# mhnazeri/PMoE

Hardware: AMD Instinct MI355X
Metric: samples/sec fwd+bwd, 256x256 RGB 4-expert PMoE (higher is better)
Workload: dtype bf16; 1 GPU; 4-expert MoE (PMoE experts), 256x256x3 x4 frames, batch 64/GPU, fwd+moe_loss+bwd, dropout 0.3; global_batch=64, parallelism=dp1

## Files before the change

### include/pmoe_hip.h

```cpp
#ifndef PMOE_HIP_H
#define PMOE_HIP_H
#include <stdint.h>
#ifdef __cplusplus
extern "C" {
#endif

#define PMOE_DT_BF16 0
#define PMOE_DT_F32 1

#define PMOE_ERR_ARG (-1)
#define PMOE_ERR_UNSUPPORTED (-2)

#define PMOE_ACT_NONE 0
#define PMOE_ACT_RELU 1
#define PMOE_ACT_ELU 2
#define PMOE_ACT_TANH 3
#define PMOE_ACT_SIGMOID 4

#define PMOE_RES_NONE 0
#define PMOE_RES_ADD 1
#define PMOE_RES_DRELU 2
#define PMOE_RES_DELU 3
#define PMOE_RES_DTANH 4
#define PMOE_RES_DSIGMOID 5
// ... 98 lines not shown
                  int64_t rows_per_expert, int32_t E, int32_t C, int32_t relu, int32_t y_ld, int32_t y_coff,
                  int32_t dtype, void* y_fp8, float in_scale, void* stream);
int pmoe_bn_apply_gap(const void* x, void* y, const float* scale, const float* shift, const float* mean, float* gap_part,
                      int32_t nparts, int32_t N, int32_t ipe, int64_t HW, int32_t C, int32_t relu, int32_t dtype, void* stream);
int pmoe_bn_bwd_reduce(const void* dy, const void* y, const void* x, const float* mean, const float* invstd,
                       const float* scale, const float* shift, int64_t rows_per_expert, int32_t E, int32_t C, int32_t relu, float* part, int32_t nparts,
                       void* gmask_out, int32_t dtype, void* stream);
int pmoe_bn_bwd_finalize(const float* part, int32_t nparts, int64_t count, float* dgamma, float* dbeta, float* c1,
                         float* c2, int32_t E, int32_t C, void* stream);
int pmoe_bn_apply_pool2(const void* x, void* y, void* pooled, const float* scale, const float* shift, const float* mean,
                        int32_t ipe, int32_t H, int32_t W, int32_t E, int32_t C, int32_t relu, int32_t y_ld, int32_t y_coff,
                        int32_t dtype, void* stream);
int pmoe_bn_bwd_apply(const void* dy, const void* y, const void* x, const float* mean, const float* invstd,
                      const float* scale, const float* shift, const float* c1, const float* c2, void* dx, void* gmask_out,
                      int64_t rows_per_expert, int32_t E, int32_t C, int32_t relu, int32_t dtype, void* stream);

int pmoe_maxpool3s2_fwd(const void* x, void* y, uint8_t* argmax, int32_t N, int32_t H, int32_t W, int32_t C,
                        int32_t dtype, void* stream);
int pmoe_maxpool3s2_bwd(const void* dy, const uint8_t* argmax, void* dx, int32_t N, int32_t H, int32_t W, int32_t C,
                        int32_t dtype, void* stream);
int pmoe_gap_partial(const void* a, const void* b, float* part, int32_t N, int64_t HW, int32_t C, int32_t nparts,
                     int32_t b_shared_ipe, int32_t dtype, void* stream);
int pmoe_gap_finish(const float* part, void* out, int32_t N, int32_t C, int32_t nparts, int64_t HW, int32_t out_ld,
                    int32_t out_coff, int32_t dtype, void* stream);
int pmoe_gap_bwd(const void* g, void* dx, int32_t N, int64_t HW, int32_t C, int32_t g_ld, int32_t g_coff,
                 int32_t dtype, void* stream);

int pmoe_stem_tail_stats(const void* z2, const float* sc2, const float* sh2, const float* mu2, float* part,
                         int32_t nparts, float* shiftc, float* part_x, int32_t E, int32_t ipe, int32_t H, int32_t W,
                         int32_t C, int32_t dtype, void* stream);
// ... 126 lines not shown
```

### pmoe_amd/csrc/elementwise.hip

```cpp
#include "common.h"

#define DISPATCH_DT(dtype, CALL)                      \
    do {                                              \
        if ((dtype) == PMOE_DT_BF16) { using T = bf16; CALL; } \
        else if ((dtype) == PMOE_DT_F32) { using T = float; CALL; } \
        else return PMOE_ERR_ARG;                     \
    } while (0)

static inline bool pow2(int v) { return v > 0 && !(v & (v - 1)); }

template <typename T, int MODE>
__global__ void __launch_bounds__(256) colstats_kernel(const T* __restrict__ x, const T* __restrict__ dy,
                                                      const T* __restrict__ y, const float* __restrict__ mean,
                                                      const float* __restrict__ invstd, const float* __restrict__ scale,
                                                      const float* __restrict__ shift, long long rpe, int C, int ld,
                                                      int coff, int relu, float* __restrict__ part, int nparts,
                                                      float* __restrict__ shiftc, T* __restrict__ gmask) {
    constexpr int VE = 16 / (int)sizeof(T);
    const int CV = C / VE, RL = 256 / CV;
    const int tid = threadIdx.x, cv = tid % CV, rl = tid / CV;
    const int e = blockIdx.y, pi = blockIdx.x;
    const long long rpp = (rpe + nparts - 1) / nparts;
    long long r0 = (long long)pi * rpp, r1 = r0 + rpp;
    if (r1 > rpe) r1 = rpe;
// ... 258 lines not shown
            for (int k = 0; k < VE; ++k) gv[k] = ((xv[k] - mu[k]) * sc[k] + sh[k]) > 0.f ? gv[k] : 0.f;
        } else if (relu) {
            float yv[VE];
            unpack16<T>(ldg16(y + off), yv);
#pragma unroll
            for (int k = 0; k < VE; ++k) gv[k] = yv[k] > 0.f ? gv[k] : 0.f;
        }
#pragma unroll
        for (int k = 0; k < VE; ++k) o[k] = gv[k] * A[k] + ((xv[k] - mu[k]) * Bx[k] + K[k]);
        stg16(dx + off, pack16<T>(o));
        if (gm) stg16(gm + off, pack16<T>(gv));
    }
}

template <typename T>
__global__ void __launch_bounds__(256) bn_apply_pool2_kernel(const T* __restrict__ x, T* __restrict__ y, T* __restrict__ pooled,
                                                            const float* __restrict__ scale, const float* __restrict__ shift,
                                                            const float* __restrict__ mean, int ipe, int H, int W, int C, int relu,
                                                            int y_ld, int y_coff) {
    constexpr int VE = 16 / (int)sizeof(T);
    const int CV = C / VE;
    const int e = blockIdx.y, Ho = H / 2, Wo = W / 2;
    const long long nq = (long long)ipe * Ho * Wo * CV;
    const long long i0 = (long long)blockIdx.x * 256 + threadIdx.x;
    const int cv = (int)(i0 % CV);
    float sc[VE], sh[VE], mu[VE];
#pragma unroll
    for (int k = 0; k < VE; ++k) {
        sc[k] = scale[e * C + cv * VE + k]; sh[k] = shift[e * C + cv * VE + k]; mu[k] = mean[e * C + cv * VE + k];
    }
// ... 500 lines not shown
                      const float* scale, const float* shift, const float* c1, const float* c2, void* dx, void* gmask_out,
                      int64_t rows_per_expert, int32_t E, int32_t C, int32_t relu, int32_t dtype, void* stream) {
    DISPATCH_DT(dtype, {
        constexpr int VE = 16 / (int)sizeof(T);
        if (C % VE || !pow2(C / VE) || C / VE > 256) return PMOE_ERR_ARG;
        const long long nvec = rows_per_expert * (C / VE);
        int cap = 1024 / (E > 0 ? E : 1);
        cap = cap < 64 ? 64 : cap;
        hipLaunchKernelGGL((bn_bwd_apply_kernel<T>), dim3(grid_for(nvec, cap), E), dim3(256), 0, (hipStream_t)stream,
                           (const T*)dy, (const T*)y, (const T*)x, mean, invstd, scale, shift, c1, c2, (T*)dx, (T*)gmask_out,
                           (long long)rows_per_expert, C, relu);
        return (int)hipGetLastError();
    });
}

int pmoe_act_fwd(const void* x, void* y, int64_t n, int32_t act, float drop_p, uint64_t seed, int32_t dtype, void* stream) {
    if (!x || !y || n <= 0 || act < PMOE_ACT_NONE || act > PMOE_ACT_SIGMOID || drop_p < 0.f || drop_p >= 1.f) return PMOE_ERR_ARG;
    DISPATCH_DT(dtype, {
        constexpr int VE = 16 / (int)sizeof(T);
        if (n % VE) return PMOE_ERR_ARG;
        hipLaunchKernelGGL((act_fwd_kernel<T>), dim3(grid_for(n / VE)), dim3(256), 0, (hipStream_t)stream, (const T*)x, (T*)y,
                           (long long)(n / VE), act, drop_p, (unsigned long long)seed);
        return (int)hipGetLastError();
    });
}

int pmoe_act_bwd(const void* dy, const void* y, void* dx, int64_t n, int32_t act, float drop_p, int32_t dtype, void* stream) {
    if (!dy || !y || !dx || n <= 0 || act < PMOE_ACT_NONE || act > PMOE_ACT_SIGMOID || drop_p < 0.f || drop_p >= 1.f) return PMOE_ERR_ARG;
    DISPATCH_DT(dtype, {
        constexpr int VE = 16 / (int)sizeof(T);
// ... 144 lines not shown
```

### pmoe_amd/engine.py

```python
import itertools
import os

import torch
import torch.distributed as dist

from . import hip, ops
from .model import blocks as B
from .parallel import BucketedAllReduce

F32 = torch.float32


def r16(c):
    return (c + 15) // 16 * 16


def r64(c):
    return (c + 63) // 64 * 64


class Var:
    __slots__ = ("t", "coff", "c", "g", "needs_grad", "act", "drop_p", "base", "gap_part", "bn_src", "bn_part", "f8", "bn_defer",
                 "bn_fused", "pending_bn")

    def __init__(self, t, c=None, coff=0, needs_grad=False, base=None):
        self.t, self.coff, self.c = t, coff, (c if c is not None else t.shape[-1])
        self.g, self.needs_grad, self.act, self.drop_p, self.base = None, needs_grad, hip.ACT_NONE, 0.0, base
        self.gap_part = None
        self.bn_src = None
        self.bn_part = None
        self.f8 = None
        self.bn_defer = False
        self.bn_fused = None
        self.pending_bn = None

    @property
    def grad(self):
        return self.base.g if self.base is not None else self.g

    def set_grad(self, g):
        if (self.base if self.base is not None else self).bn_part is not None:
            raise RuntimeError("relu(BatchNorm(z)) whose backward reductions came out of its consumer's data gradient "
                               "(PMOE_RES_DBN) must have exactly one consumer; a second gradient contribution arrived "
                               "(set PMOE_BN_REDUCE_IN_DGRAD=0 for graphs that fan this activation out)")
        if self.base is not None:
            self.base.g = g
        else:
            self.g = g

# ... 139 lines not shown
        self._built_for = self._ptr_key = self._packed_version = None
        self._build_gen = 0
        self._seed_counter = itertools.count(1)
        self.fuse_conv_stats = True
        self.fuse_stem_tail = True
        self.fold_stem_input = True
        self.overlap_wgrad = os.environ.get("PMOE_OVERLAP_WGRAD", "0") == "1"
        self.fold_bn_eval = True
        self.pooled_stem_bwd = True
        self.fold_eca_gate = True
        self.bn_mask_in_reduce = os.environ.get("PMOE_BN_MASK_IN_REDUCE", "1") != "0"
        self.bn_reduce_in_dgrad = os.environ.get("PMOE_BN_REDUCE_IN_DGRAD", "1") != "0"
        self.fuse_bn_gap = os.environ.get("PMOE_FUSE_BN_GAP", "1") != "0"
        self.stem_bn_fuse = os.environ.get("PMOE_STEM_BN_FUSE", "1") != "0"
        self.mlp_wgrad_fused = os.environ.get("PMOE_MLP_WGRAD", "1") != "0"
        self.fp8 = False
        self.fp8_in_scale = 16.0
        self.fp8_min_cin = int(os.environ.get("PMOE_FP8_MIN_CIN", "64"))
        self.raw_alpha = False
        self.debug_grads = None
        self.debug_acts = None
        self._collect()

    def _collect(self):
        ex = self.experts
        self.params = []
        self.all_convs = []

        def conv(name, mods, ks=None):
            m0 = mods[0]
# ... 334 lines not shown
            if part is None:
                nparts = self._nparts(rpe)
                part = torch.empty(E, nparts, 2, C_, dtype=F32, device=self.dev)
                shiftc = torch.empty(E, C_, dtype=F32, device=self.dev)
                ops.colstats(rpe, z.t, E, C_, part, nparts, shiftc=shiftc)
            part, nparts = self._fold_parts(part, nparts, 2 * C_, cap=2048)
            ops.bn_finalize(part, nparts, rpe, self._tab("gamma", layer), self._tab("beta", layer),
                            self._tab("rm", layer), self._tab("rv", layer), layer.momentum, layer.eps, True, scale,
                            shift, mean, invstd, E, C_, shiftc)
            self._bn_touched.append(layer)
        else:
            ops.bn_finalize(scale, 0, rpe, self._tab("gamma", layer), self._tab("beta", layer), self._tab("rm", layer),
                            self._tab("rv", layer), layer.momentum, layer.eps, False, scale, shift, mean, invstd, E, C_)
        return scale, shift, mean, invstd

    def _bn(self, z, layer, relu, res=None, stats=None, out=None, out_coff=0, want_gap=False, want_f8=False, pool_to=None):
        E, C_ = self.E, layer.C
        n, h, w, _ = z.t.shape
        rpe = self.B * h * w
        if stats is not None and stats.shape[2] != C_:
            raise RuntimeError("fused stats width mismatch")
        scale, shift, mean, invstd = self._bn_coeffs(layer, rpe, stats, stats.shape[0] // E if stats is not None else 0, z)
        if out is None:
            y = Var(torch.empty_like(z.t))
        elif self.taping:
            y = Var(out.t, C_, out_coff)
        else:
            y = out.window(out_coff, C_)
        ops.set_meta(name=layer.name, bytes=z.t.numel() * z.t.element_size() * (3 if res is not None else 2))
        if want_gap and res is None and out is None and self.fuse_bn_gap:
            nparts = self._gap_parts(h * w)
            part = torch.empty(n, nparts, C_, dtype=F32, device=self.dev)
            ops.bn_apply_gap(z.t, y.t, scale, shift, mean, part, nparts, self.B, relu)
            y.gap_part = (part, nparts)
        elif pool_to is not None and res is None:
            ops.bn_apply_pool2(z.t, y.t, pool_to, scale, shift, mean, self.B, E, C_, relu, y_coff=y.coff)
        else:
            if want_f8 and out is None and self.dtype == torch.bfloat16:
                y.f8 = torch.empty(y.t.shape, dtype=torch.uint8, device=self.dev)
            ops.bn_apply(z.t, res.t if res is not None else None, y.t, scale, shift, mean, rpe, E, C_, relu, y_coff=y.coff,
                         y_fp8=y.f8, in_scale=self.fp8_in_scale)
        if self.debug_acts is not None and relu:
            self.debug_acts[layer.name] = (y.t, y.coff, C_)
        if (relu and res is None and out is None and self.taping and self.training and self.bn_reduce_in_dgrad
                and self.dtype == torch.bfloat16 and z.needs_grad):
            y.bn_src = (z, layer, self._last_coef, rpe)
        y.needs_grad = z.needs_grad or layer.trainable or (res is not None and res.needs_grad)
        if out is not None and y.needs_grad:
            out.needs_grad = True
        if self.taping and y.needs_grad:
            train = self.training
            self.tape.append(lambda: self._bn_bwd(z, layer, y, res, relu, scale, shift, mean, invstd, rpe, train))
        return y

    def _bn_bwd(self, z, layer, y, res, relu, scale, shift, mean, invstd, rpe, train):
        dy = y.grad
# ... 10 lines not shown
                raise RuntimeError("BatchNorm reductions from the data-gradient epilogue: channel count mismatch")
            part, nparts = self._fold_parts(part.view(E, nparts, 2 * C_), nparts, 2 * C_, cap=2048)
            c1, c2 = self._bn_bwd_finalize(layer, part, nparts, rpe, train)
            if z.needs_grad:
                if z.grad is not None:
                    raise RuntimeError("BN input consumed twice")
                if z.bn_defer:
                    z.bn_fused = (dy, y.bn_src[2], c1, c2)
                    z.set_grad(dy)
                    return
                dz = torch.empty_like(z.t)
                ops.set_meta(name=layer.name, bytes=nb * 3)
                ops.bn_bwd_apply(dy, None, z.t, mean, invstd, scale, shift, c1, c2, dz, None, rpe, E, C_, False)
                z.set_grad(dz)
            return
        nparts = self._nparts(rpe)
        part = torch.empty(E, nparts, 2, C_, dtype=F32, device=self.dev)
        want_res = res is not None and res.needs_grad
        gm = torch.empty_like(z.t) if (want_res and relu and ysrc is not None and self.bn_mask_in_reduce) else None
        ops.set_meta(name=layer.name, bytes=nb * ((3 if ysrc is not None else 2) + (gm is not None)))
        ops.bn_bwd_reduce(dy, ysrc, z.t, mean, invstd, scale, shift, rpe, E, C_, relu, part, nparts, gmask=gm)
        part, nparts = self._fold_parts(part, nparts, 2 * C_, cap=2048)
        c1, c2 = self._bn_bwd_finalize(layer, part, nparts, rpe, train)
        dz = torch.empty_like(z.t) if z.needs_grad else None
        if gm is not None:
            if dz is not None:
                ops.set_meta(name=layer.name, bytes=nb * 3)
                ops.bn_bwd_apply(gm, None, z.t, mean, invstd, scale, shift, c1, c2, dz, None, rpe, E, C_, False)
        else:
            gm = torch.empty_like(z.t) if want_res else None
# ... 2 lines not shown
            if dz is None:
                dz = torch.empty_like(z.t)
            ops.set_meta(name=layer.name, bytes=nb * (2 + (ysrc is not None) + 1 + (gm is not None)))
            ops.bn_bwd_apply(dy, ysrc, z.t, mean, invstd, scale, shift, c1, c2, dz, gm, rpe, E, C_, relu)
        if self.debug_grads is not None:
            self.debug_grads[layer.name + ":dz"] = dz.detach().clone()
            self.debug_grads[layer.name + ":stats"] = (mean.clone(), invstd.clone(), c1.clone(), c2.clone())
        if z.needs_grad:
            if z.grad is not None:
                raise RuntimeError("BN input consumed twice")
            z.set_grad(dz)
        if want_res:
            if res.grad is not None:
                raise RuntimeError("residual gradient slot already filled")
            res.set_grad(gm)

    def _bn_bwd_finalize(self, layer, part, nparts, rpe, train, out=None):
        E, C_ = self.E, layer.C
        c1, c2 = out or (torch.empty(E, C_, dtype=F32, device=self.dev) for _ in range(2))
        dgamma, dbeta, store = self._bn_grad_views(layer)
        ops.bn_bwd_finalize(part, nparts, rpe, dgamma, dbeta, c1, c2, E, C_)
        if store is not None:
            store()
        if not train:
            c1.zero_()
            c2.zero_()
        return c1, c2

    def _bn_grad_views(self, layer):
        return (self._grad_slot("gamma", layer).view(self.E, layer.C), self._grad_slot("beta", layer).view(self.E, layer.C),
# ... 327 lines not shown
            a1 = self._conv_bn(x0s, self.conv1, self.bn_c1, relu=True)
        if fold2:
            z2, st = self._eca_conv_folded(a1, self.eca2, self.conv2)
        else:
            a1s = self._eca(a1, self.eca2, shared=False)
            z2, st = self._conv_stats(a1s, self.conv2)
        if self.fuse_stem_tail:
            o = self._stem_tail(z2, st)
        else:
            a2 = self._bn(z2, self.bn_c2, relu=True, stats=st)
            a3 = self._bn(a2, self.bn1, relu=True)
            o = self._maxpool(a3)
        for bi, blk in enumerate(self.blocks):
            idn = o
            if blk["down"] is not None:
                idn = self._conv_bn(o, blk["down"][0], blk["down"][1], relu=False)
            nxt = self.blocks[bi + 1]["conv1"] if bi + 1 < len(self.blocks) else None
            aA = self._conv_bn(o, blk["conv1"], blk["bn1"], relu=True, want_f8=blk["conv2"].fp8)
            o = self._conv_bn(aA, blk["conv2"], blk["bn2"], relu=True, res=idn, want_f8=nxt is not None and nxt.fp8)
        self._gap_to(o, feat, 0)

    def _conv_bn(self, x, conv, bn, relu, res=None, out=None, want_f8=False, pool_to=None):
        if self.training or self.taping or not self.fold_bn_eval or conv.w_f8 is not None:
            z, st = self._conv_stats(x, conv)
            return self._bn(z, bn, relu=relu, res=res, stats=st, out=out, want_f8=want_f8, pool_to=pool_to)
        E = self.E
        key = (self.dtype, str(self.dev)) + tuple(p._version for p in conv.weights) + tuple(
            v for m in bn.mods for v in (m.weight._version, m.bias._version, m.running_mean._version, m.running_var._version))
        cache = conv.__dict__.get("_bn_fold")
        if cache is None or cache[0] != key:
            scale, shift, mean, _ = self._bn_coeffs(bn, 1)
            wf = torch.empty(E, conv.coutp, conv.taps, conv.cinp, dtype=self.dtype, device=self.dev)
            bf = torch.empty(E, conv.coutp, dtype=F32, device=self.dev)
            ops.pack_conv_weights_scaled(self._tab("w", conv), scale, shift, mean, wf, bf, E, conv.cout, conv.cin, conv.ks,
                                         conv.coutp, conv.cinp, self.dtype)
            cache = conv.__dict__["_bn_fold"] = (key, wf, bf)
        _, wf, bf = cache
        Ho, Wo, o = self._conv_out(x, conv, out)
        ops.set_meta(flop=2.0 * self.N * Ho * Wo * conv.cout * conv.cin * conv.taps, name=conv.name + "+bn")
        ops.conv2d(x.t, wf, o.t, cin=conv.cinp, cout=conv.cout_st, coutp=conv.coutp, ipe=self.B, ks=conv.ks,
# ... 173 lines not shown
```

### pmoe_amd/engine_punet.py

```python
import os
import types

import torch

from . import hip, ops
from .engine import ExpertGroupEngine, GroupedBN, GroupedConv, Var, r16, F32


class _UpConv(GroupedConv):
    route_bias = False

    def __init__(self, eng, name, mod):
        super().__init__(eng, name, None, None, mod.in_channels, 4 * mod.out_channels, 1, 1, 0)
        self.mod, self.c_up = mod, mod.out_channels
        self.need_dgrad = False
        self.biases = [mod.bias]
        self._derived_version = None

    @property
    def trainable(self):
        return self.mod.weight.requires_grad or self.mod.bias.requires_grad

    def scatter_grads(self, eng, full_w, full_b):
        eng._grad_slot("wT", self).view(self.cin, self.c_up, 2, 2).copy_(
# ... 10 lines not shown
                              self.cinp, self.dg_rows, self.dg_red, self.w_fwd.dtype)
        ops.pack_bias(hip.ptr_table([b], dev), self.bias_packed, 1, self.cout, self.coutp)
        self._derived_version = ver


class PUNetEngine(ExpertGroupEngine):
    _punet_trains = False

    def __init__(self, expert, return_inter=None):
        self.return_inter = expert.return_inter if return_inter is None else return_inter
        self._punet_built_for, self._punet_build_gen = None, 0
        self.debug_pass_out = self.debug_forced_masks = None
        self.debug_x0 = self.debug_x0_kept = None
        self.debug_keep_x0 = False
        super().__init__([expert], alt=False)

    def _collect_pre_backbone(self, ex):
        pu = ex[0].punet
        self.pu = pu
        self.up_layers = []
        self.shadow_bns = []
        self.unet = self._collect_unet("punet.unet", pu.unet)
        conv, bn, eca = self._mk["conv"], self._mk["bn"], self._mk["eca"]
        eb = pu.entry_block
        self.entry = dict(eca1=eca("punet.entry.eca1", [eb.layer1.eca1]),
                          conv1=conv("punet.entry.conv1", [eb.layer1.conv1[0]]),
                          bn1=bn("punet.entry.bn1", [eb.layer1.conv1[1]]),
                          eca2=eca("punet.entry.eca2", [eb.layer2.eca2]),
                          conv2=conv("punet.entry.conv2", [eb.layer2.conv2[0]]),
                          bn2=self._padded_bn("punet.entry.bn2", eb.layer2.conv2[1]))
# ... 604 lines not shown
```

### pmoe_amd/hip.py

```python
import ctypes as C
import os
from pathlib import Path

import torch

_LIB_PATH = Path(os.environ.get("PMOE_HIP_LIB") or Path(__file__).resolve().parent / "libpmoe_hip.so")
_lib = None

ABI_VERSION = 401
DT_BF16, DT_F32 = 0, 1
ACT_NONE, ACT_RELU, ACT_ELU, ACT_TANH, ACT_SIGMOID = 0, 1, 2, 3, 4
RES_NONE, RES_ADD, RES_DRELU, RES_DELU, RES_DTANH, RES_DSIGMOID, RES_DBN, RES_INBN = 0, 1, 2, 3, 4, 5, 6, 7
ERR_ARG, ERR_UNSUPPORTED = -1, -2
RES_OF_ACT = {ACT_RELU: RES_DRELU, ACT_ELU: RES_DELU, ACT_TANH: RES_DTANH, ACT_SIGMOID: RES_DSIGMOID}
ACT_BY_NAME = {"relu": ACT_RELU, "elu": ACT_ELU, "tanh": ACT_TANH, "sigmoid": ACT_SIGMOID}

_TORCH_DT = {torch.bfloat16: DT_BF16, torch.float32: DT_F32}


class HipUnavailable(RuntimeError):
    pass


class ConvDesc(C.Structure):
# ... 46 lines not shown
    "pmoe_pack_conv_weights": [_P, _P, _P, _I, _I, _I, _I, _I, _I, _I, _I, _I, _P],
    "pmoe_pack_conv_weights_fp8": [_P, _P, _P, _P, _P, _F, _I, _I, _I, _I, _I, _I, _I, _I, _P],
    "pmoe_pack_conv_weights_scaled": [_P, _P, _P, _P, _P, _P, _I, _I, _I, _I, _I, _I, _I, _P],
    "pmoe_pack_conv_weights_gated": [_P, _P, _I, _P, _P, _I, _I, _I, _I, _I, _I, _I, _I, _I, _I, _P],
    "pmoe_unpack_conv_wgrad": [_P, _P, _I, _I, _I, _I, _I, _I, _P],
    "pmoe_pack_bias": [_P, _P, _I, _I, _I, _P],
    "pmoe_act_fwd": [_P, _P, _L, _I, _F, C.c_uint64, _I, _P],
    "pmoe_act_bwd": [_P, _P, _P, _L, _I, _F, _I, _P],
    "pmoe_colstats": [_P, _L, _I, _I, _I, _I, _P, _I, _P, _I, _P],
    "pmoe_reduce_partials": [_P, _P, _I, _I, _I, _I, _P],
    "pmoe_bn_finalize": [_P, _I, _L, _P, _P, _P, _P, _F, _F, _I, _P, _P, _P, _P, _I, _I, _P, _P],
    "pmoe_bn_apply": [_P, _P, _P, _P, _P, _P, _L, _I, _I, _I, _I, _I, _I, _P, _F, _P],
    "pmoe_bn_bwd_reduce": [_P, _P, _P, _P, _P, _P, _P, _L, _I, _I, _I, _P, _I, _P, _I, _P],
    "pmoe_bn_bwd_finalize": [_P, _I, _L, _P, _P, _P, _P, _I, _I, _P],
    "pmoe_bn_bwd_apply": [_P, _P, _P, _P, _P, _P, _P, _P, _P, _P, _P, _L, _I, _I, _I, _I, _P],
    "pmoe_stem_tail_stats": [_P, _P, _P, _P, _P, _I, _P, _P, _I, _I, _I, _I, _I, _I, _P],
    "pmoe_stem_tail_pooled": [_P, _P, _P, C.POINTER(C.c_void_p), _P, _I, _I, _L, _I, _I, _P],
    "pmoe_stem_tail_combine": [_P, _I, _P, _I, C.POINTER(C.c_void_p), _L, _P, _P, _I, _I, _P],
    "pmoe_stem_tail_pool": [_P, _P, _P, _P, _P, _P, _P, _P, _P, _I, _I, _I, _I, _I, _I, _P],
    "pmoe_stem_tail_bwd": [_I, _P, _P, _P, _P, C.POINTER(C.c_void_p), _P, _I, _I, _I, _I, _I, _I, _I, _P],
    "pmoe_maxpool3s2_fwd": [_P, _P, _P, _I, _I, _I, _I, _I, _P],
    "pmoe_maxpool3s2_bwd": [_P, _P, _P, _I, _I, _I, _I, _I, _P],
    "pmoe_gap_partial": [_P, _P, _P, _I, _L, _I, _I, _I, _I, _P],
    "pmoe_bn_apply_gap": [_P, _P, _P, _P, _P, _P, _I, _I, _I, _L, _I, _I, _I, _P],
    "pmoe_gap_finish": [_P, _P, _I, _I, _I, _L, _I, _I, _I, _P],
    "pmoe_gap_bwd": [_P, _P, _I, _L, _I, _I, _I, _I, _P],
    "pmoe_eca_gate": [_P, _I, _L, _P, _I, _P, _P, _I, _I, _I, _I, _I, _P],
    "pmoe_eca_scale": [_P, _P, _P, _I, _L, _I, _I, _I, _P],
    "pmoe_eca_bwd_small": [_P, _I, _P, _P, _P, _I, _P, _P, _P, _I, _I, _I, _I, _F, _P],
    "pmoe_eca_stem_fold": [_P, _P, _P, _P, _P, _I, _I, _I, _I, _I, _I, _I, _I, _P],
# ... 148 lines not shown
```

### pmoe_amd/ops.py

```python
import ctypes as C

import torch

from . import hip
from .hip import ConvDesc, WgradDesc, check, dt, load, ptr, stream_ptr


def _round_up(v, m):
    return (v + m - 1) // m * m


def conv_out_size(h, ks, stride, pad):
    return (h + 2 * pad - ks) // stride + 1


def _nhwc(t, name):
    if t.dim() != 4:
        raise ValueError(f"{name}: expected NHWC [N,H,W,C], got shape {tuple(t.shape)}")
    return t.shape


def _conv_desc(n, h, w_, ho, wo, cin, cout, coutp, ipe, ks, stride, pad, dtype, *, dilate=False, in_shared=False, in_ld=0,
               in_coff=0, out_ld=0, out_coff=0, res_mode=hip.RES_NONE, res_ld=0, res_coff=0, act=hip.ACT_NONE, drop_p=0.0, seed=0,
               w_fp8=False, in_fp8=False, in_scale=1.0, bn_ipe=0, shuffle2_c=0):
# ... 264 lines not shown
                                    ptr(scale), ptr(shift), rpe, E, C_, int(relu), ptr(part, "part", torch.float32), nparts,
                                    ptr(gmask, "gmask", dy.dtype), dt(dy), stream_ptr()), "pmoe_bn_bwd_reduce")


def bn_bwd_finalize(part, nparts, count, dgamma, dbeta, c1, c2, E, C_):
    check(load().pmoe_bn_bwd_finalize(ptr(part), nparts, count, ptr(dgamma), ptr(dbeta), ptr(c1), ptr(c2), E, C_,
                                      stream_ptr()), "pmoe_bn_bwd_finalize")


def bn_bwd_apply(dy, y, x, mean, invstd, scale, shift, c1, c2, dx, gmask, rpe, E, C_, relu):
    check(load().pmoe_bn_bwd_apply(ptr(dy, "dy"), ptr(y, "y", dy.dtype), ptr(x, "x", dy.dtype), ptr(mean), ptr(invstd),
                                   ptr(scale), ptr(shift), ptr(c1), ptr(c2), ptr(dx, "dx", dy.dtype), ptr(gmask, "gmask", dy.dtype),
                                   rpe, E, C_, int(relu), dt(dy), stream_ptr()), "pmoe_bn_bwd_apply")


def stem_tail_stats(z2, sc2, sh2, mu2, part, nparts, E, ipe, shiftc=None, part_x=None):
    n, h, w_, c = _nhwc(z2, "z2")
    check(load().pmoe_stem_tail_stats(ptr(z2, "z2"), ptr(sc2), ptr(sh2), ptr(mu2), ptr(part, "part", torch.float32), nparts,
                                      ptr(shiftc, "shiftc", torch.float32), ptr(part_x, "part_x", torch.float32), E, ipe,
                                      h, w_, c, dt(z2), stream_ptr()), "pmoe_stem_tail_stats")


def _consts12(consts):
    return (C.c_void_p * 12)(*[t.data_ptr() if t is not None else None for t in consts])


def stem_tail_pooled(y, dpool, argmax, consts, part4, nparts, E):
    n, ho, wo, c = _nhwc(y, "y")
    check(load().pmoe_stem_tail_pooled(ptr(y, "y"), ptr(dpool, "dpool", y.dtype), ptr(argmax, "argmax", torch.uint8),
                                       _consts12(consts), ptr(part4, "part4", torch.float32), nparts, E,
# ... 164 lines not shown
        meta, _next_meta = _next_meta, {}
        e0, e1 = torch.cuda.Event(enable_timing=True), torch.cuda.Event(enable_timing=True)
        e0.record()
        r = fn(*a, **k)
        e1.record()
        if _launch_info:
            meta.update(_launch_info)
            _launch_info.clear()
        _prof.append((fn.__name__, meta, e0, e1))
        return r
    return wrapper


for _n in ("stem_tail_stats", "stem_tail_pool", "stem_tail_bwd", "stem_tail_pooled", "stem_tail_combine", "conv2d", "conv2d_wgrad", "conv2d_wgrad_fold", "pack_conv_weights", "pack_conv_weights_scaled", "pack_conv_weights_gated", "unpack_conv_wgrad", "pack_bias", "colstats",
           "reduce_partials", "bn_finalize", "bn_apply", "bn_apply_gap", "bn_bwd_reduce", "bn_bwd_finalize", "bn_bwd_apply",
           "maxpool_fwd", "maxpool_bwd", "gap_partial", "gap_finish", "gap_bwd", "eca_gate", "eca_scale",
           "eca_bwd_small", "eca_bwd_apply", "eca_stem_fold", "nchw_to_nhwc", "pad_rows", "gate_mixture_fwd", "gate_mixture_bwd",
           "moe_loss"):
    globals()[_n] = _timed(globals()[_n])


def maxpool2_fwd(x, y, c=None, x_coff=0):
    n, h, w_, ld = _nhwc(x, "x")
    c = ld if c is None else c
    if tuple(y.shape) != (n, h // 2, w_ // 2, c):
        raise ValueError(f"maxpool2_fwd: y must be {(n, h // 2, w_ // 2, c)}, got {tuple(y.shape)}")
    check(load().pmoe_maxpool2s2_fwd(ptr(x, "x"), ptr(y, "y", x.dtype), n, h, w_, c, ld, x_coff, dt(x), stream_ptr()),
          "pmoe_maxpool2s2_fwd")


# ... 217 lines not shown
```

Baseline: 1953 samples/s.

## Fold shortcut downsample BatchNorm into residual block's BN apply and backward

Defers the downsample-branch BatchNorm during training, so the shortcut's normalized tensor is never materialized. The block's second BN applies both normalizations in one pass (bn_apply_pair). Backward uses paired reduce and apply kernels that compute both BNs' gradient statistics and input gradients from one read of the shared masked gradient. This removes a separate BN apply pass plus one backward pass and several launches per downsample block. The cost is more registers and shared memory per kernel, and tighter shape constraints enforced at runtime.

```diff
diff --git a/include/pmoe_hip.h b/include/pmoe_hip.h
--- a/include/pmoe_hip.h
+++ b/include/pmoe_hip.h
@@ -136,6 +136,16 @@
 int pmoe_bn_bwd_apply(const void* dy, const void* y, const void* x, const float* mean, const float* invstd,
                       const float* scale, const float* shift, const float* c1, const float* c2, void* dx, void* gmask_out,
                       int64_t rows_per_expert, int32_t E, int32_t C, int32_t relu, int32_t dtype, void* stream);
+int pmoe_bn_apply_pair(const void* x, const void* xd, void* y, const float* scale, const float* shift, const float* mean,
+                       const float* scale_d, const float* shift_d, const float* mean_d, int64_t rows_per_expert, int32_t E,
+                       int32_t C, int32_t relu, int32_t dtype, void* y_fp8, float in_scale, void* stream);
+int pmoe_bn_bwd_reduce_pair(const void* dy, const void* y, const void* x, const void* xd, const float* mean,
+                            const float* invstd, const float* mean_d, const float* invstd_d, int64_t rows_per_expert, int32_t E,
+                            int32_t C, float* part, float* part_d, int32_t nparts, void* gmask_out, int32_t dtype, void* stream);
+int pmoe_bn_bwd_apply_pair(const void* g, const void* x, const void* xd, const float* mean, const float* invstd,
+                           const float* scale, const float* c1, const float* c2, const float* mean_d, const float* invstd_d,
+                           const float* scale_d, const float* c1_d, const float* c2_d, void* dx, void* dxd,
+                           int64_t rows_per_expert, int32_t E, int32_t C, int32_t dtype, void* stream);
 
 int pmoe_maxpool3s2_fwd(const void* x, void* y, uint8_t* argmax, int32_t N, int32_t H, int32_t W, int32_t C,
                         int32_t dtype, void* stream);
diff --git a/pmoe_amd/csrc/elementwise.hip b/pmoe_amd/csrc/elementwise.hip
--- a/pmoe_amd/csrc/elementwise.hip
+++ b/pmoe_amd/csrc/elementwise.hip
@@ -296,6 +296,164 @@
 }
 
 template <typename T>
+__global__ void __launch_bounds__(256) bn_apply_pair_kernel(const T* __restrict__ x, const T* __restrict__ xd, T* __restrict__ y,
+                                                           const float* __restrict__ scale, const float* __restrict__ shift,
+                                                           const float* __restrict__ mean, const float* __restrict__ scale_d,
+                                                           const float* __restrict__ shift_d, const float* __restrict__ mean_d,
+                                                           long long rpe, int C, int relu, unsigned char* __restrict__ y8,
+                                                           float in_scale) {
+    constexpr int VE = 16 / (int)sizeof(T);
+    const int CV = C / VE;
+    const int e = blockIdx.y;
+    const long long nvec = rpe * CV;
+    const size_t ebase = (size_t)e * rpe * C;
+    const long long i0 = (long long)blockIdx.x * 256 + threadIdx.x;
+    const int cv = (int)(i0 % CV);
+    float sc[VE], sh[VE], mu[VE], scd[VE], shd[VE], mud[VE];
+#pragma unroll
+    for (int k = 0; k < VE; ++k) {
+        const int c = e * C + cv * VE + k;
+        sc[k] = scale[c]; sh[k] = shift[c]; mu[k] = mean[c];
+        scd[k] = scale_d[c]; shd[k] = shift_d[c]; mud[k] = mean_d[c];
+    }
+    for (long long i = i0; i < nvec; i += (long long)gridDim.x * 256) {
+        float xv[VE], rv[VE];
+        const size_t off = ebase + (size_t)i * VE;
+        unpack16<T>(ldg16(x + off), xv);
+        unpack16<T>(ldg16(xd + off), rv);
+#pragma unroll
+        for (int k = 0; k < VE; ++k) rv[k] = (rv[k] - mud[k]) * scd[k] + shd[k];
+        unpack16<T>(pack16<T>(rv), rv);
+#pragma unroll
+        for (int k = 0; k < VE; ++k) xv[k] = (xv[k] - mu[k]) * sc[k] + sh[k];
+#pragma unroll
+        for (int k = 0; k < VE; ++k) xv[k] += rv[k];
+        if (relu) {
+#pragma unroll
+            for (int k = 0; k < VE; ++k) xv[k] = fmaxf(xv[k], 0.f);
+        }
+        const v4i pk = pack16<T>(xv);
+        stg16(y + off, pk);
+        if constexpr (sizeof(T) == 2) {
+            if (y8) {
+                float q[VE];
+                unpack16<T>(pk, q);
+                int w0 = 0, w1 = 0;
+#pragma unroll
+                for (int k = 0; k < VE; ++k) q[k] = fminf(fmaxf(q[k] * in_scale, -PMOE_FP8_MAX), PMOE_FP8_MAX);
+                w0 = __builtin_amdgcn_cvt_pk_fp8_f32(q[0], q[1], w0, false);
+                w0 = __builtin_amdgcn_cvt_pk_fp8_f32(q[2], q[3], w0, true);
+                w1 = __builtin_amdgcn_cvt_pk_fp8_f32(q[4], q[5], w1, false);
+                w1 = __builtin_amdgcn_cvt_pk_fp8_f32(q[6], q[7], w1, true);
+                *reinterpret_cast<int2*>(y8 + off) = int2{w0, w1};
+            }
+        }
+    }
+}
+
+template <typename T>
+__global__ void __launch_bounds__(256) bn_bwd_reduce_pair_kernel(const T* __restrict__ x, const T* __restrict__ xd,
+                                                                const T* __restrict__ dy, const T* __restrict__ y,
+                                                                const float* __restrict__ mean, const float* __restrict__ invstd,
+                                                                const float* __restrict__ mean_d, const float* __restrict__ invstd_d,
+                                                                long long rpe, int C, float* __restrict__ part,
+                                                                float* __restrict__ part_d, int nparts, T* __restrict__ gmask) {
+    constexpr int VE = 16 / (int)sizeof(T);
+    const int CV = C / VE, RL = 256 / CV;
+    const int tid = threadIdx.x, cv = tid % CV, rl = tid / CV;
+    const int e = blockIdx.y, pi = blockIdx.x;
+    const long long rpp = (rpe + nparts - 1) / nparts;
+    long long r0 = (long long)pi * rpp, r1 = r0 + rpp;
+    if (r1 > rpe) r1 = rpe;
+    float s1[VE], s2[VE], t2[VE], mu[VE], is[VE], mud[VE], isd[VE];
+#pragma unroll
+    for (int i = 0; i < VE; ++i) {
+        const int c = e * C + cv * VE + i;
+        s1[i] = s2[i] = t2[i] = 0.f;
+        mu[i] = mean[c]; is[i] = invstd[c];
+        mud[i] = mean_d[c]; isd[i] = invstd_d[c];
+    }
+    const size_t ebase = (size_t)e * rpe;
+    for (long long r = r0 + rl; r < r1; r += RL) {
+        const size_t off = (ebase + r) * C + cv * VE;
+        float xv[VE], dv[VE], gv[VE], yv[VE];
+        unpack16<T>(ldg16(x + off), xv);
+        unpack16<T>(ldg16(xd + off), dv);
+        unpack16<T>(ldg16(dy + off), gv);
+        unpack16<T>(ldg16(y + off), yv);
+#pragma unroll
+        for (int i = 0; i < VE; ++i) gv[i] = yv[i] > 0.f ? gv[i] : 0.f;
+        stg16(gmask + off, pack16<T>(gv));
+#pragma unroll
+        for (int i = 0; i < VE; ++i) {
+            s1[i] += gv[i];
+            s2[i] += gv[i] * (xv[i] - mu[i]) * is[i];
+            t2[i] += gv[i] * (dv[i] - mud[i]) * isd[i];
+        }
+    }
+    __shared__ float red[3][256 * 8];
+#pragma unroll
+    for (int i = 0; i < VE; ++i) {
+        red[0][rl * C + cv * VE + i] = s1[i];
+        red[1][rl * C + cv * VE + i] = s2[i];
+        red[2][rl * C + cv * VE + i] = t2[i];
+    }
+    __syncthreads();
+    for (int c = tid; c < 3 * C; c += 256) {
+        const int which = c / C, cc = c % C;
+        float s = 0.f;
+        for (int k = 0; k < RL; ++k) s += red[which][k * C + cc];
+        const size_t row = ((size_t)e * nparts + pi) * 2;
+        if (which < 2) part[(row + which) * C + cc] = s;
+        if (which != 1) part_d[(row + which / 2) * C + cc] = s;
+    }
+}
+
+template <typename T>
+__global__ void __launch_bounds__(256) bn_bwd_apply_pair_kernel(const T* __restrict__ g, const T* __restrict__ x,
+                                                               const T* __restrict__ xd, const float* __restrict__ mean,
+                                                               const float* __restrict__ invstd, const float* __restrict__ scale,
+                                                               const float* __restrict__ c1, const float* __restrict__ c2,
+                                                               const float* __restrict__ mean_d, const float* __restrict__ invstd_d,
+                                                               const float* __restrict__ scale_d, const float* __restrict__ c1_d,
+                                                               const float* __restrict__ c2_d, T* __restrict__ dx,
+                                                               T* __restrict__ dxd, long long rpe, int C) {
+    constexpr int VE = 16 / (int)sizeof(T);
+    const int CV = C / VE;
+    const int e = blockIdx.y;
+    const long long nvec = rpe * CV;
+    const size_t ebase = (size_t)e * rpe * C;
+    const long long i0 = (long long)blockIdx.x * 256 + threadIdx.x;
+    const int cv = (int)(threadIdx.x & (CV - 1));
+    float A[VE], Bx[VE], K[VE], mu[VE], Ad[VE], Bxd[VE], Kd[VE], mud[VE];
+#pragma unroll
+    for (int k = 0; k < VE; ++k) {
+        const int c = e * C + cv * VE + k;
+        mu[k] = mean[c];
+        A[k] = scale[c];
+        Bx[k] = -A[k] * invstd[c] * c2[c];
+        K[k] = -A[k] * c1[c];
+        mud[k] = mean_d[c];
+        Ad[k] = scale_d[c];
+        Bxd[k] = -Ad[k] * invstd_d[c] * c2_d[c];
+        Kd[k] = -Ad[k] * c1_d[c];
+    }
+    for (long long i = i0; i < nvec; i += (long long)gridDim.x * 256) {
+        const size_t off = ebase + (size_t)i * VE;
+        float gv[VE], xv[VE], dv[VE], o[VE];
+        unpack16<T>(ldg16(g + off), gv);
+        unpack16<T>(ldg16(x + off), xv);
+        unpack16<T>(ldg16(xd + off), dv);
+#pragma unroll
+        for (int k = 0; k < VE; ++k) o[k] = gv[k] * A[k] + ((xv[k] - mu[k]) * Bx[k] + K[k]);
+        stg16(dx + off, pack16<T>(o));
+#pragma unroll
+        for (int k = 0; k < VE; ++k) o[k] = gv[k] * Ad[k] + ((dv[k] - mud[k]) * Bxd[k] + Kd[k]);
+        stg16(dxd + off, pack16<T>(o));
+    }
+}
+
+template <typename T>
 __global__ void __launch_bounds__(256) bn_apply_pool2_kernel(const T* __restrict__ x, T* __restrict__ y, T* __restrict__ pooled,
                                                             const float* __restrict__ scale, const float* __restrict__ shift,
                                                             const float* __restrict__ mean, int ipe, int H, int W, int C, int relu,
@@ -826,6 +984,59 @@
     });
 }
 
+int pmoe_bn_apply_pair(const void* x, const void* xd, void* y, const float* scale, const float* shift, const float* mean,
+                       const float* scale_d, const float* shift_d, const float* mean_d, int64_t rows_per_expert, int32_t E,
+                       int32_t C, int32_t relu, int32_t dtype, void* y_fp8, float in_scale, void* stream) {
+    if (!x || !xd || !y || !scale || !shift || !mean || !scale_d || !shift_d || !mean_d || rows_per_expert < 1 || E < 1)
+        return PMOE_ERR_ARG;
+    if (y_fp8 && dtype != PMOE_DT_BF16) return PMOE_ERR_ARG;
+    DISPATCH_DT(dtype, {
+        constexpr int VE = 16 / (int)sizeof(T);
+        if (C % VE || !pow2(C / VE) || C / VE > 256) return PMOE_ERR_ARG;
+        const long long nvec = rows_per_expert * (C / VE);
+        hipLaunchKernelGGL((bn_apply_pair_kernel<T>), dim3(grid_for(nvec, 2048), E), dim3(256), 0, (hipStream_t)stream,
+                           (const T*)x, (const T*)xd, (T*)y, scale, shift, mean, scale_d, shift_d, mean_d,
+                           (long long)rows_per_expert, C, relu, (unsigned char*)y_fp8, in_scale);
+        return (int)hipGetLastError();
+    });
+}
+
+int pmoe_bn_bwd_reduce_pair(const void* dy, const void* y, const void* x, const void* xd, const float* mean,
+                            const float* invstd, const float* mean_d, const float* invstd_d, int64_t rows_per_expert, int32_t E,
+                            int32_t C, float* part, float* part_d, int32_t nparts, void* gmask_out, int32_t dtype, void* stream) {
+    if (!dy || !y || !x || !xd || !mean || !invstd || !mean_d || !invstd_d || !part || !part_d || !gmask_out ||
+        rows_per_expert < 1 || E < 1 || nparts < 1)
+        return PMOE_ERR_ARG;
+    DISPATCH_DT(dtype, {
+        constexpr int VE = 16 / (int)sizeof(T);
+        if (C % VE || !pow2(C / VE) || C / VE > 256) return PMOE_ERR_ARG;
+        hipLaunchKernelGGL((bn_bwd_reduce_pair_kernel<T>), dim3(nparts, E), dim3(256), 0, (hipStream_t)stream, (const T*)x,
+                           (const T*)xd, (const T*)dy, (const T*)y, mean, invstd, mean_d, invstd_d, (long long)rows_per_expert,
+                           C, part, part_d, nparts, (T*)gmask_out);
+        return (int)hipGetLastError();
+    });
+}
+
+int pmoe_bn_bwd_apply_pair(const void* g, const void* x, const void* xd, const float* mean, const float* invstd,
+                           const float* scale, const float* c1, const float* c2, const float* mean_d, const float* invstd_d,
+                           const float* scale_d, const float* c1_d, const float* c2_d, void* dx, void* dxd,
+                           int64_t rows_per_expert, int32_t E, int32_t C, int32_t dtype, void* stream) {
+    if (!g || !x || !xd || !mean || !invstd || !scale || !c1 || !c2 || !mean_d || !invstd_d || !scale_d || !c1_d || !c2_d ||
+        !dx || !dxd || rows_per_expert < 1 || E < 1)
+        return PMOE_ERR_ARG;
+    DISPATCH_DT(dtype, {
+        constexpr int VE = 16 / (int)sizeof(T);
+        if (C % VE || !pow2(C / VE) || C / VE > 256) return PMOE_ERR_ARG;
+        const long long nvec = rows_per_expert * (C / VE);
+        int cap = 1024 / E;
+        cap = cap < 64 ? 64 : cap;
+        hipLaunchKernelGGL((bn_bwd_apply_pair_kernel<T>), dim3(grid_for(nvec, cap), E), dim3(256), 0, (hipStream_t)stream,
+                           (const T*)g, (const T*)x, (const T*)xd, mean, invstd, scale, c1, c2, mean_d, invstd_d, scale_d, c1_d,
+                           c2_d, (T*)dx, (T*)dxd, (long long)rows_per_expert, C);
+        return (int)hipGetLastError();
+    });
+}
+
 int pmoe_act_fwd(const void* x, void* y, int64_t n, int32_t act, float drop_p, uint64_t seed, int32_t dtype, void* stream) {
     if (!x || !y || n <= 0 || act < PMOE_ACT_NONE || act > PMOE_ACT_SIGMOID || drop_p < 0.f || drop_p >= 1.f) return PMOE_ERR_ARG;
     DISPATCH_DT(dtype, {
diff --git a/pmoe_amd/engine.py b/pmoe_amd/engine.py
--- a/pmoe_amd/engine.py
+++ b/pmoe_amd/engine.py
@@ -21,7 +21,7 @@
 
 class Var:
     __slots__ = ("t", "coff", "c", "g", "needs_grad", "act", "drop_p", "base", "gap_part", "bn_src", "bn_part", "f8", "bn_defer",
-                 "bn_fused", "pending_bn")
+                 "bn_fused", "pending_bn", "down_bn")
 
     def __init__(self, t, c=None, coff=0, needs_grad=False, base=None):
         self.t, self.coff, self.c = t, coff, (c if c is not None else t.shape[-1])
@@ -33,6 +33,7 @@
         self.bn_defer = False
         self.bn_fused = None
         self.pending_bn = None
+        self.down_bn = None
 
     @property
     def grad(self):
@@ -202,6 +203,7 @@
         self.fuse_bn_gap = os.environ.get("PMOE_FUSE_BN_GAP", "1") != "0"
         self.stem_bn_fuse = os.environ.get("PMOE_STEM_BN_FUSE", "1") != "0"
         self.mlp_wgrad_fused = os.environ.get("PMOE_MLP_WGRAD", "1") != "0"
+        self.fold_down_bn = os.environ.get("PMOE_DOWN_BN_FOLD", "1") != "0"
         self.fp8 = False
         self.fp8_in_scale = 16.0
         self.fp8_min_cin = int(os.environ.get("PMOE_FP8_MIN_CIN", "64"))
@@ -566,13 +568,20 @@
                             self._tab("rv", layer), layer.momentum, layer.eps, False, scale, shift, mean, invstd, E, C_)
         return scale, shift, mean, invstd
 
-    def _bn(self, z, layer, relu, res=None, stats=None, out=None, out_coff=0, want_gap=False, want_f8=False, pool_to=None):
+    def _bn(self, z, layer, relu, res=None, stats=None, out=None, out_coff=0, want_gap=False, want_f8=False, pool_to=None,
+            defer=False):
         E, C_ = self.E, layer.C
         n, h, w, _ = z.t.shape
         rpe = self.B * h * w
         if stats is not None and stats.shape[2] != C_:
             raise RuntimeError("fused stats width mismatch")
         scale, shift, mean, invstd = self._bn_coeffs(layer, rpe, stats, stats.shape[0] // E if stats is not None else 0, z)
+        if defer:
+            z.down_bn = (layer, scale, shift, mean, invstd)
+            return z
+        down = res.down_bn if res is not None else None
+        if down is not None and (not relu or out is not None or res.t.shape != z.t.shape or down[0].C != C_):
+            raise RuntimeError(f"{layer.name}: a deferred shortcut BatchNorm needs relu(bn + shortcut) into a dense output of its own shape")
         if out is None:
             y = Var(torch.empty_like(z.t))
         elif self.taping:
@@ -590,8 +599,12 @@
         else:
             if want_f8 and out is None and self.dtype == torch.bfloat16:
                 y.f8 = torch.empty(y.t.shape, dtype=torch.uint8, device=self.dev)
-            ops.bn_apply(z.t, res.t if res is not None else None, y.t, scale, shift, mean, rpe, E, C_, relu, y_coff=y.coff,
-                         y_fp8=y.f8, in_scale=self.fp8_in_scale)
+            if down is not None:
+                ops.bn_apply_pair(z.t, res.t, y.t, scale, shift, mean, down[1], down[2], down[3], rpe, E, C_, relu,
+                                  y_fp8=y.f8, in_scale=self.fp8_in_scale)
+            else:
+                ops.bn_apply(z.t, res.t if res is not None else None, y.t, scale, shift, mean, rpe, E, C_, relu, y_coff=y.coff,
+                             y_fp8=y.f8, in_scale=self.fp8_in_scale)
         if self.debug_acts is not None and relu:
             self.debug_acts[layer.name] = (y.t, y.coff, C_)
         if (relu and res is None and out is None and self.taping and self.training and self.bn_reduce_in_dgrad
@@ -632,6 +645,8 @@
                 ops.bn_bwd_apply(dy, None, z.t, mean, invstd, scale, shift, c1, c2, dz, None, rpe, E, C_, False)
                 z.set_grad(dz)
             return
+        if res is not None and res.down_bn is not None:
+            return self._bn_bwd_pair(z, layer, y, res, scale, mean, invstd, rpe, train)
         nparts = self._nparts(rpe)
         part = torch.empty(E, nparts, 2, C_, dtype=F32, device=self.dev)
         want_res = res is not None and res.needs_grad
@@ -664,6 +679,30 @@
             if res.grad is not None:
                 raise RuntimeError("residual gradient slot already filled")
             res.set_grad(gm)
+
+    def _bn_bwd_pair(self, z, layer, y, zd, scale, mean, invstd, rpe, train):
+        dlayer, dscale, _, dmean, dinvstd = zd.down_bn
+        if z.grad is not None or zd.grad is not None:
+            raise RuntimeError("BN input consumed twice")
+        E, C_ = self.E, layer.C
+        nb = z.t.numel() * z.t.element_size()
+        nparts = self._nparts(rpe)
+        part = torch.empty(2, E, nparts, 2, C_, dtype=F32, device=self.dev)
+        gm = torch.empty_like(z.t)
+        ops.set_meta(name=layer.name, bytes=nb * 5)
+        ops.bn_bwd_reduce_pair(y.grad, y.t, z.t, zd.t, mean, invstd, dmean, dinvstd, rpe, E, C_, part[0], part[1], nparts, gm)
+        c1, c2 = self._bn_bwd_finalize(layer, *self._fold_parts(part[0], nparts, 2 * C_, cap=2048), rpe, train)
+        d1, d2 = self._bn_bwd_finalize(dlayer, *self._fold_parts(part[1], nparts, 2 * C_, cap=2048), rpe, train)
+        dz, dzd = torch.empty_like(z.t), torch.empty_like(z.t)
+        ops.set_meta(name=layer.name, bytes=nb * 5)
+        ops.bn_bwd_apply_pair(gm, z.t, zd.t, mean, invstd, scale, c1, c2, dmean, dinvstd, dscale, d1, d2, dz, dzd, rpe, E, C_)
+        if self.debug_grads is not None:
+            self.debug_grads[dlayer.name] = gm.detach().clone()
+            for name, g_, st in ((layer.name, dz, (mean, invstd, c1, c2)), (dlayer.name, dzd, (dmean, dinvstd, d1, d2))):
+                self.debug_grads[name + ":dz"] = g_.detach().clone()
+                self.debug_grads[name + ":stats"] = tuple(t.clone() for t in st)
+        z.set_grad(dz)
+        zd.set_grad(dzd)
 
     def _bn_bwd_finalize(self, layer, part, nparts, rpe, train, out=None):
         E, C_ = self.E, layer.C
@@ -1021,16 +1060,17 @@
         for bi, blk in enumerate(self.blocks):
             idn = o
             if blk["down"] is not None:
-                idn = self._conv_bn(o, blk["down"][0], blk["down"][1], relu=False)
+                idn = self._conv_bn(o, blk["down"][0], blk["down"][1], relu=False,
+                                    defer=self.fold_down_bn and self.training and self.taping and o.needs_grad)
             nxt = self.blocks[bi + 1]["conv1"] if bi + 1 < len(self.blocks) else None
             aA = self._conv_bn(o, blk["conv1"], blk["bn1"], relu=True, want_f8=blk["conv2"].fp8)
             o = self._conv_bn(aA, blk["conv2"], blk["bn2"], relu=True, res=idn, want_f8=nxt is not None and nxt.fp8)
         self._gap_to(o, feat, 0)
 
-    def _conv_bn(self, x, conv, bn, relu, res=None, out=None, want_f8=False, pool_to=None):
+    def _conv_bn(self, x, conv, bn, relu, res=None, out=None, want_f8=False, pool_to=None, defer=False):
         if self.training or self.taping or not self.fold_bn_eval or conv.w_f8 is not None:
             z, st = self._conv_stats(x, conv)
-            return self._bn(z, bn, relu=relu, res=res, stats=st, out=out, want_f8=want_f8, pool_to=pool_to)
+            return self._bn(z, bn, relu=relu, res=res, stats=st, out=out, want_f8=want_f8, pool_to=pool_to, defer=defer)
         E = self.E
         key = (self.dtype, str(self.dev)) + tuple(p._version for p in conv.weights) + tuple(
             v for m in bn.mods for v in (m.weight._version, m.bias._version, m.running_mean._version, m.running_var._version))
diff --git a/pmoe_amd/engine_punet.py b/pmoe_amd/engine_punet.py
--- a/pmoe_amd/engine_punet.py
+++ b/pmoe_amd/engine_punet.py
@@ -48,6 +48,7 @@
         self.debug_x0 = self.debug_x0_kept = None
         self.debug_keep_x0 = False
         super().__init__([expert], alt=False)
+        self.fold_down_bn = False
 
     def _collect_pre_backbone(self, ex):
         pu = ex[0].punet
diff --git a/pmoe_amd/hip.py b/pmoe_amd/hip.py
--- a/pmoe_amd/hip.py
+++ b/pmoe_amd/hip.py
@@ -84,6 +84,9 @@
     "pmoe_bn_bwd_reduce": [_P, _P, _P, _P, _P, _P, _P, _L, _I, _I, _I, _P, _I, _P, _I, _P],
     "pmoe_bn_bwd_finalize": [_P, _I, _L, _P, _P, _P, _P, _I, _I, _P],
     "pmoe_bn_bwd_apply": [_P, _P, _P, _P, _P, _P, _P, _P, _P, _P, _P, _L, _I, _I, _I, _I, _P],
+    "pmoe_bn_apply_pair": [_P, _P, _P, _P, _P, _P, _P, _P, _P, _L, _I, _I, _I, _I, _P, _F, _P],
+    "pmoe_bn_bwd_reduce_pair": [_P, _P, _P, _P, _P, _P, _P, _P, _L, _I, _I, _P, _P, _I, _P, _I, _P],
+    "pmoe_bn_bwd_apply_pair": [_P, _P, _P, _P, _P, _P, _P, _P, _P, _P, _P, _P, _P, _P, _P, _L, _I, _I, _I, _P],
     "pmoe_stem_tail_stats": [_P, _P, _P, _P, _P, _I, _P, _P, _I, _I, _I, _I, _I, _I, _P],
     "pmoe_stem_tail_pooled": [_P, _P, _P, C.POINTER(C.c_void_p), _P, _I, _I, _L, _I, _I, _P],
     "pmoe_stem_tail_combine": [_P, _I, _P, _I, C.POINTER(C.c_void_p), _L, _P, _P, _I, _I, _P],
diff --git a/pmoe_amd/ops.py b/pmoe_amd/ops.py
--- a/pmoe_amd/ops.py
+++ b/pmoe_amd/ops.py
@@ -302,6 +302,41 @@
                                    rpe, E, C_, int(relu), dt(dy), stream_ptr()), "pmoe_bn_bwd_apply")
 
 
+def bn_apply_pair(x, xd, y, scale, shift, mean, scale_d, shift_d, mean_d, rpe, E, C_, relu, y_fp8=None, in_scale=1.0):
+    if y_fp8 is not None and (y_fp8.dtype != torch.uint8 or y_fp8.shape != y.shape):
+        raise ValueError("bn_apply_pair: y_fp8 must be a uint8 tensor of y's shape")
+    if xd.shape != x.shape or y.shape != x.shape:
+        raise ValueError("bn_apply_pair: x, xd and y must have one shape")
+    f32 = torch.float32
+    check(load().pmoe_bn_apply_pair(ptr(x, "x"), ptr(xd, "xd", x.dtype), ptr(y, "y", x.dtype), ptr(scale, "scale", f32),
+                                    ptr(shift, "shift", f32), ptr(mean, "mean", f32), ptr(scale_d, "scale_d", f32),
+                                    ptr(shift_d, "shift_d", f32), ptr(mean_d, "mean_d", f32), rpe, E, C_, int(relu), dt(x),
+                                    ptr(y_fp8, "y_fp8", torch.uint8), float(in_scale), stream_ptr()), "pmoe_bn_apply_pair")
+
+
+def bn_bwd_reduce_pair(dy, y, x, xd, mean, invstd, mean_d, invstd_d, rpe, E, C_, part, part_d, nparts, gmask):
+    if not (dy.shape == y.shape == x.shape == xd.shape == gmask.shape) or part.shape != part_d.shape:
+        raise ValueError("bn_bwd_reduce_pair: dy, y, x, xd, gmask must have one shape, part and part_d another")
+    f32 = torch.float32
+    check(load().pmoe_bn_bwd_reduce_pair(ptr(dy, "dy"), ptr(y, "y", dy.dtype), ptr(x, "x", dy.dtype), ptr(xd, "xd", dy.dtype),
+                                         ptr(mean, "mean", f32), ptr(invstd, "invstd", f32), ptr(mean_d, "mean_d", f32),
+                                         ptr(invstd_d, "invstd_d", f32), rpe, E, C_, ptr(part, "part", f32),
+                                         ptr(part_d, "part_d", f32), nparts, ptr(gmask, "gmask", dy.dtype), dt(dy),
+                                         stream_ptr()), "pmoe_bn_bwd_reduce_pair")
+
+
+def bn_bwd_apply_pair(g, x, xd, mean, invstd, scale, c1, c2, mean_d, invstd_d, scale_d, c1_d, c2_d, dx, dxd, rpe, E, C_):
+    if not (g.shape == x.shape == xd.shape == dx.shape == dxd.shape):
+        raise ValueError("bn_bwd_apply_pair: g, x, xd, dx, dxd must have one shape")
+    f32 = torch.float32
+    check(load().pmoe_bn_bwd_apply_pair(ptr(g, "g"), ptr(x, "x", g.dtype), ptr(xd, "xd", g.dtype), ptr(mean, "mean", f32),
+                                        ptr(invstd, "invstd", f32), ptr(scale, "scale", f32), ptr(c1, "c1", f32),
+                                        ptr(c2, "c2", f32), ptr(mean_d, "mean_d", f32), ptr(invstd_d, "invstd_d", f32),
+                                        ptr(scale_d, "scale_d", f32), ptr(c1_d, "c1_d", f32), ptr(c2_d, "c2_d", f32),
+                                        ptr(dx, "dx", g.dtype), ptr(dxd, "dxd", g.dtype), rpe, E, C_, dt(g), stream_ptr()),
+          "pmoe_bn_bwd_apply_pair")
+
+
 def stem_tail_stats(z2, sc2, sh2, mu2, part, nparts, E, ipe, shiftc=None, part_x=None):
     n, h, w_, c = _nhwc(z2, "z2")
     check(load().pmoe_stem_tail_stats(ptr(z2, "z2"), ptr(sc2), ptr(sh2), ptr(mu2), ptr(part, "part", torch.float32), nparts,
@@ -496,6 +531,7 @@
 
 for _n in ("stem_tail_stats", "stem_tail_pool", "stem_tail_bwd", "stem_tail_pooled", "stem_tail_combine", "conv2d", "conv2d_wgrad", "conv2d_wgrad_fold", "pack_conv_weights", "pack_conv_weights_scaled", "pack_conv_weights_gated", "unpack_conv_wgrad", "pack_bias", "colstats",
            "reduce_partials", "bn_finalize", "bn_apply", "bn_apply_gap", "bn_bwd_reduce", "bn_bwd_finalize", "bn_bwd_apply",
+           "bn_apply_pair", "bn_bwd_reduce_pair", "bn_bwd_apply_pair",
            "maxpool_fwd", "maxpool_bwd", "gap_partial", "gap_finish", "gap_bwd", "eca_gate", "eca_scale",
            "eca_bwd_small", "eca_bwd_apply", "eca_stem_fold", "nchw_to_nhwc", "pad_rows", "gate_mixture_fwd", "gate_mixture_bwd",
            "moe_loss"):
```

After: 1987 samples/s, median of 6. 1.7% higher.
